# ninjasource/lc3-codec

Hardware: AMD Instinct MI355X
Metric: LC3 frames/sec (encode+decode) @48kHz/10ms (higher is better)
Workload: dtype f32

## Files before the change

### lc3-codec_amd/csrc/lc3_dev_common.h

```cpp
#pragma once
#include <stddef.h>
#include <stdint.h>

#include "lc3_dev_experiments.h"

#define LC3_TABLE_QUAL static __device__ const
#include "../../tables/lc3_tables.h"

#ifndef LC3_STAMP
#define LC3_STAMP(L, lane, id)
#endif

#ifndef LC3_CFG_PARAM
#define LC3_CFG_TEMPLATE
#define LC3_CFG_TEMPLATE_AND(...) template <__VA_ARGS__>
#define LC3_CFG_PARAM const lc3_cfg &c
#define LC3_CFG_BIND
#define LC3_CFG_PASS c
#endif

#ifndef LC3_LDS_PARAM
#define LC3_LDS_DECL(T, arr)
#define LC3_LDS_PARAM(T) T &L,
#define LC3_LDS_PASS L,
// ... 14 lines not shown
            (void)sub;
#define LC3_SERIAL_END \
        }              \
        LC3_SYNC();    \
    }
#endif
#ifndef LC3_SERIAL_WIDE_BEGIN
#define LC3_SERIAL_WIDE_BEGIN(T, L, lane, phase, K) LC3_SERIAL_BEGIN(T, L, lane, phase, K)
#endif

#define LC3_LOCAL_BEGIN(lane, K)    \
    {                               \
        LC3_SYNC();                 \
        if ((lane) < (K)) {         \
            const int sub = (lane); \
            (void)sub;
#define LC3_LOCAL_END \
        }             \
        LC3_SYNC();   \
    }

#ifndef LC3_KEEP_SCALAR
#define LC3_KEEP_SCALAR(x) ((void)0)
#endif
#ifndef LC3_UNIFORM_I32
#define LC3_UNIFORM_I32(x) (x)
#endif
#ifndef LC3_KEEP_PER_FRAME
#define LC3_KEEP_PER_FRAME(x) ((void)0)
#endif
#ifndef LC3_UNIFORM_PTR
#define LC3_UNIFORM_PTR(T, p) ((T)(p))
#endif
#ifndef LC3_LDS_BASE
#define LC3_LDS_BASE(p) (p)
#endif
#ifndef LC3_LDS_BASE_ALIGNED
#define LC3_LDS_BASE_ALIGNED(p, bytes) (p)
#endif
#ifndef LC3_HBM_CONST
#define LC3_HBM_CONST(T) const T *
#define LC3_HBM(T) T *
#endif

#define LC3_WAVE 64
#ifndef LC3_LOCKSTEP
// ... 885 lines not shown
```

### lc3-codec_amd/csrc/lc3_dev_enc.h

```cpp
#pragma once
#include "lc3_dev_common.h"
#include "lc3_dev_enc_pack.h"
#include "lc3_dev_enc_vq.h"

struct lc3_enc_scalars {
    float att_energy_last, att_max_energy_last;
    int att_pos_last, att_ds_tm1, att_ds_tm2;
    int t_prev;
    float mem_pitch;
    int mem_ltpf_active;
    float mem_nc, mem_mem_nc, h50_m1, h50_m2;
    int reset_offset_old;
    float nbits_offset_old;
    int nbits_est_old;
    int nbits_spec_old;
    int ring12_head, ring6_head, pad_[2];
};
struct lc3_enc_state {
    float x12[384];
    float x6[180];
    int16_t hist[304];
    lc3_enc_scalars sc;
};
static_assert(sizeof(lc3_enc_scalars) == 80 && sizeof(lc3_enc_state) % 16 == 0 && offsetof(lc3_enc_state, sc) % 16 == 0,
// ... 1 lines not shown

struct __attribute__((aligned(16))) lc3_enc_lds {
    lc3_enc_scalars st;
    float spec[LC3_MAX_NF];
    lc3_cpx fa[LC3_MAX_NF / 2];
    lc3_cpx fb[LC3_MAX_NF / 2];
    int16_t t[2 * LC3_MAX_NF];
    float sm[32];
    int ism[64];
    int spec_flags;
    int pad_;
    unsigned long long prof_last;
#ifdef LC3_PROFILE
    unsigned long long prof_acc[32];
#endif
};
#define LC3_ENC_DBG_EB 1472
#define LC3_ENC_DBG_ATTACK 1536
#define LC3_ENC_DBG_FLOATS 1600
#define LC3_EB(L) ((float *)(L).fa + 512)
#define LC3_SCF(L) ((float *)(L).fa + 144)
#define LC3_XQ(L) ((L).t)
#define LC3_RESW(L) ((uint32_t *)((uint8_t *)(L).t + 1024))

LC3_LDS_DECL(lc3_enc_lds, lc3_enc_wg)
static_assert(offsetof(lc3_enc_lds, fa) % 16 == 0 && offsetof(lc3_enc_lds, spec) % 16 == 0 && offsetof(lc3_enc_lds, t) % 16 == 0,
              "128-bit LDS reads need aligned buffers");
#ifndef LC3_PROFILE
static_assert(sizeof(lc3_enc_lds) <= 8192, "encoder working set: 8 KB per stream (the kernels run 16 waves per CU, register-bound)");
#endif

struct lc3_tns_res { int nbits_tns, lpc_weighting, num_tns_filters; int rc_order[2]; };
struct lc3_ltpf_res { int pitch_index, pitch_present, ltpf_active, nbits_ltpf; };
struct lc3_quant_res { int gg_ind, nbits_spec, nbits_lsb, nbits_trunc, lsb_mode, rate_flag, lastnz_trunc; float gg; };

#ifndef LC3_HBM_FENCE
#define LC3_HBM_FENCE() LC3_SYNC()
#endif

__device__ __forceinline__ void lc3_enc_state_init(lc3_enc_lds &L, int lane, lc3_enc_state *g, int valid) {
    int *w = (int *)&L.st;
    if (lane < (int)(sizeof(lc3_enc_scalars) / 4)) w[lane] = 0;
    if (valid) {
        int *gw = (int *)g;
        for (int i = lane; i < (int)(offsetof(lc3_enc_state, sc) / 4); i += LC3_WAVE) gw[i] = 0;
    }
// ... 333 lines not shown
        if (attack) {
            sSCF[0] = (sDS[0] + sDS[1] + sDS[2]) / 3.0f;
            sSCF[1] = (sDS[0] + sDS[1] + sDS[2] + sDS[3]) / 4.0f;
            for (int n = 2; n < 14; n++) {
                float wt = 0.0f;
                for (int k = n - 2; k < n + 3; k++) wt += sDS[k];
                sSCF[n] = wt / 5.0f;
            }
            sSCF[14] = (sDS[12] + sDS[13] + sDS[14] + sDS[15]) / 4.0f;
            sSCF[15] = (sDS[13] + sDS[14] + sDS[15]) / 3.0f;
            total = 0.0f;
            for (int n = 0; n < 16; n++) total += sSCF[n];
            avg = total / 16.0f;
            const float att = c.n_ms_10 ? 0.5f : 0.3f;
            for (int n = 0; n < 16; n++) sSCF[n] = att * (sSCF[n] - avg);
        } else {
            for (int n = 0; n < 16; n++) sSCF[n] = sDS[n];
        }
    }
    LC3_SYNC();
    LC3_STAMP(L, lane, 27);
}

#define LC3_TNS_CHUNK 4
struct lc3_tns_slot {
    float q[54];
    float es[6];
    int p_bw, near_nyquist, on[2];
    float rc[16];
};
static_assert(sizeof(lc3_tns_slot) * LC3_TNS_CHUNK <= sizeof(((lc3_enc_lds *)0)->fb), "the slots live in fb, which the back half does not use otherwise");
#define LC3_TNS_SLOT(L, u) (((lc3_tns_slot *)(L).fb)[(u)])

LC3_CFG_TEMPLATE __device__ __noinline__ void lc3_enc_tns_acf(LC3_CFG_PARAM, LC3_LDS_PARAM(lc3_enc_lds) int lane, int p_bw, int near_nyquist,
                                              int slot) {
    LC3_CFG_BIND;
    LC3_LDS_BIND(lc3_enc_lds, lc3_enc_wg);
    const lc3_tns_params &tp = c.n_ms_10 ? LC3C_TNS10[p_bw] : LC3C_TNS75[p_bw];
    lc3_tns_slot &T = LC3_TNS_SLOT(L, slot);
    float *sAC = T.q, *sES = T.es;
    float *x = L.spec;
    const int ne = c.ne;
    LC3_ENC_REPEAT(16) {
    if ((lane & 31) < 27) {
        const int j = (lane & 31) / 9, k = (lane & 31) - 9 * j;
        const int blk = lane < 32 ? (j == 2 ? 3 : j) : (j == 0 ? 2 : j + 3);
        const int f = blk >= 3, s = blk - 3 * f;
        float ac = 0.0f;
        if (f < tp.num) {
            const int start = tp.sub_start[f][s], stop = tp.sub_stop[f][s], k_from = start + k;
            if (k_from < ne && k_from < stop) {
                const float *pa = x + start, *pb = x + k_from;
                const int n = stop - k_from;
                for (int i = 0; i < n; i += 8) {
                    float xa[8], xb[8];
#pragma unroll
                    for (int u = 0; u < 8; u++) {
                        xa[u] = pa[i + u];
                        xb[u] = pb[i + u];
                    }
                    if (i + 8 <= n) {
#pragma unroll
                        for (int u = 0; u < 8; u++) ac += xa[u] * xb[u];
                    } else {
#pragma unroll
                        for (int u = 0; u < 8; u++) {
                            const float p = xa[u] * xb[u];
                            ac = i + u < n ? ac + p : ac;
                        }
                    }
                }
            }
        }
        sAC[f * 27 + k * 3 + s] = ac;
        if (k == 0) sES[f * 3 + s] = ac;
    }
    if (lane == 0) {
        T.p_bw = p_bw;
        T.near_nyquist = near_nyquist;
    }
    LC3_SYNC();
    if (lane < 54) {
        const int f = lane / 27, r = lane - 27 * f, s3 = r - 3 * (r / 3);
        sAC[lane] = sAC[lane] / sES[f * 3 + s3];
    }
    LC3_SYNC();
    }
    LC3_STAMP(L, lane, 28);
}

LC3_CFG_TEMPLATE __device__ __noinline__ void lc3_enc_tns_lev(LC3_CFG_PARAM, LC3_LDS_PARAM(lc3_enc_lds) int lane, int nbits, int n) {
    LC3_CFG_BIND;
    LC3_LDS_BIND(lc3_enc_lds, lc3_enc_wg);
    const int lpc_weighting = c.n_ms_10 ? (nbits < 480) : (nbits < 360);
    LC3_ENC_REPEAT(32)
    if (lane < 2 * n) {
        const int f = lane & 1;
        lc3_tns_slot &T = LC3_TNS_SLOT(L, lane >> 1);
        const float *sAC = T.q, *sES = T.es;
        float *rc_q = T.rc;
        const int num_g = (c.n_ms_10 ? LC3C_TNS10[T.p_bw] : LC3C_TNS75[T.p_bw]).num;
        int on = 0;
        if (f < num_g) {
        float r[9];
        const float e_prod = (1.0f * sES[f * 3] * sES[f * 3 + 1]) * sES[f * 3 + 2];
#pragma unroll
        for (int k = 0; k < 9; k++) {
            const float r0 = k == 0 ? 3.0f : 0.0f;
            const float rk = ((0.0f + sAC[f * 27 + k * 3]) + sAC[f * 27 + k * 3 + 1]) + sAC[f * 27 + k * 3 + 2];
            r[k] = (e_prod == 0.0f ? r0 : rk) * LC3C_TNS_LAGW[k];
        }
// ... 760 lines not shown
            LC3_GUARD_ASSERT((acc <= fits && nbits_spec >= 0) == ((int)lc3_ceilf((float)acc / 2048.0f) <= nbits_spec));
            cand_k = ok ? k0 + j : cand_k;
            cand_est = ok ? acc : cand_est;
        }
        const int best_k = lc3_wave_max_i32(cand_k, lane);
        const uint32_t best_est = best_k >= 0 ? (uint32_t)lc3_wave_read_i32((int)cand_est, best_k >> 2, lane) : 0u;
        bc.lastnz = lastnz;
        bc.lastnz_trunc = best_k < 0 ? 2 : 2 * best_k + 2;
        bc.nbits_est = (int)lc3_ceilf((float)est_total / 2048.0f) + (int)lsb_total;
        bc.nbits_trunc = (int)lc3_ceilf((float)best_est / 2048.0f);
        bc.nbits_lsb = (int)lsb_total;
    }
    (void)ntup_all;
    bc.rate_flag = rate_flag;
    bc.mode_flag = mode_flag;
    LC3_SYNC();
    for (int n = bc.lastnz_trunc + lane; n < bc.lastnz; n += LC3_WAVE) LC3_XQ(L)[n] = 0;
    LC3_SYNC();
    bc.lsb_mode = bc.mode_flag && bc.nbits_est > nbits_spec;
    bc.gg = gg;
    return bc;
}

LC3_CFG_TEMPLATE __device__ __noinline__ lc3_quant_res lc3_enc_quant(LC3_CFG_PARAM, LC3_LDS_PARAM(lc3_enc_lds) int lane, int nbits, int nbits_bw,
                                                      int nbits_tns, int nbits_ltpf) {
    LC3_CFG_BIND;
    LC3_LDS_BIND(lc3_enc_lds, lc3_enc_wg);
    const int ne = c.ne, ne4 = ne / 4;
    lc3_quant_res res;
    int nbits_ari = 0;
    while ((1 << nbits_ari) < ne / 2) nbits_ari++;
    nbits_ari += nbits <= 1280 ? 3 : (nbits <= 2560 ? 4 : 5);
    const int nbits_spec = nbits - (nbits_bw + nbits_tns + nbits_ltpf + 38 + 8 + 3 + nbits_ari);
    float nbits_offset;
    if (L.st.reset_offset_old) nbits_offset = 0.0f;
    else {
        float prev = L.st.nbits_offset_old + (float)L.st.nbits_spec_old - (float)L.st.nbits_est_old;
        nbits_offset = 0.8f * L.st.nbits_offset_old + 0.2f * lc3_minf(40.0f, lc3_maxf(-40.0f, prev));
    }
    const int nbits_spec_adj = lc3_f2u16((float)nbits_spec + nbits_offset + 0.5f);
    int gg_off;
    {
        int q = (int)(int16_t)nbits / (10 * (c.fs_ind + 1));
        gg_off = -(q < 115 ? q : 115) - 105 - 5 * (c.fs_ind + 1);
    }
    float e14[2], e28[2], amax = 0.0f;
    const lc3_divisor by20 = lc3_divisor_make(20.0f);
    LC3_ENC_REPEAT(1)
#pragma unroll
    for (int q = 0; q < 2; q++) {
        const int n = lane + LC3_WAVE * q;
        const lc3_f4 x = *(const lc3_f4 *)(L.spec + 4 * (n < ne4 ? n : 0));
// ... 85 lines not shown
        if (L.spec_flags & LC3_SPEC_NBITS_SPEC_OLD) L.st.nbits_spec_old = nbits_spec;
        L.st.reset_offset_old = reset_offset;
    }
    {
        const int t1 = LC3C_GGA_T1[c.fs_ind], t2 = LC3C_GGA_T2[c.fs_ind], t3 = LC3C_GGA_T3[c.fs_ind], est = bc.nbits_est, origin = gg_ind;
        float delta;
        if (est < t1) delta = ((float)est + 48.0f) / 16.0f;
        else if (est < t2) {
            float tmp1 = (float)t1 / 16.0f + 3.0f, tmp2 = (float)t2 / 48.0f;
            delta = ((float)est - (float)t1) * (tmp2 - tmp1) / ((float)t2 - (float)t1) + tmp1;
        } else if (est < t3) delta = (float)est / 48.0f;
        else delta = (float)t3 / 48.0f;
        delta = lc3_floorf(delta + 0.5f);
        const float delta2 = delta + 2.0f;
        if ((gg_ind < 255 && est > nbits_spec) || (gg_ind > 0 && (float)est < ((float)nbits_spec - delta2))) {
            if ((float)est < ((float)nbits_spec - delta2)) gg_ind -= 1;
            else if (gg_ind == 254 || (float)est < ((float)nbits_spec + delta)) gg_ind += 1;
            else gg_ind += 2;
            if (gg_ind < gg_min) gg_ind = gg_min;
        }
        if (origin != gg_ind)
            LC3_ENC_REPEAT(8) bc = lc3_quantize_spectrum(LC3_CFG_PASS, LC3_LDS_PASS lane, nbits, gg_off, gg_ind, nbits_spec);
    }
    res.gg_ind = gg_ind;
    res.nbits_spec = nbits_spec;
    res.nbits_lsb = bc.nbits_lsb;
    res.lsb_mode = bc.lsb_mode;
    res.nbits_trunc = bc.nbits_trunc;
    res.rate_flag = bc.rate_flag;
    res.lastnz_trunc = bc.lastnz_trunc;
    res.gg = bc.gg;
    return res;
}

LC3_CFG_TEMPLATE __device__ __noinline__ int lc3_enc_residual_noise(LC3_CFG_PARAM, LC3_LDS_PARAM(lc3_enc_lds) int lane,
                                                    const lc3_quant_res q, int bw_ind) {
    LC3_CFG_BIND;
    LC3_LDS_BIND(lc3_enc_lds, lc3_enc_wg);
    const int ne = c.ne;
    float *compact = (float *)L.fa;
    const int bw_stop = c.n_ms_10 ? LC3C_BWSTOP10[bw_ind] : LC3C_BWSTOP75[bw_ind];
    const int nf_start = c.n_ms_10 ? 24 : 18, nf_width = c.n_ms_10 ? 3 : 2;
    const int nf_stop = ne < bw_stop ? ne : bw_stop;
    int mx = q.nbits_spec - q.nbits_trunc + 4;
    if (mx < 0) mx = 0;
    const int k0 = 8 * lane;
    int xv[8];
    float sv[8];
    {
        const lc3_i4 w = *(const lc3_i4 *)(LC3_XQ(L) + k0);
        const lc3_f4 sa = *(const lc3_f4 *)(L.spec + k0), sb = *(const lc3_f4 *)(L.spec + k0 + 4);
        int wi[4];
        __builtin_memcpy(wi, &w, 16);
#pragma unroll
        for (int i = 0; i < 4; i++) {
// ... 220 lines not shown
        float *d = dbg + 1440;
        d[0] = (float)bw_ind; d[1] = (float)attack; d[9] = (float)pf.pitch_index; d[10] = (float)pf.pitch_present;
        d[11] = (float)pf.ltpf_active; d[21] = (float)near_nyquist;
        float *a = dbg + LC3_ENC_DBG_ATTACK;
        a[0] = L.st.att_energy_last; a[1] = L.st.att_max_energy_last; a[2] = (float)L.st.att_pos_last;
        a[3] = (float)L.st.att_ds_tm1; a[4] = (float)L.st.att_ds_tm2;
    }
    if (plane && mid && lane == 0) {
        const int st = plane_stride;
        int32_t *mf = (int32_t *)mid + MP_FLAGS;
        mf[MPF_BW] = bw_ind;
        mf[MPF_NBITS_BW] = nbits_bw;
        mf[MPF_NEAR_NYQUIST] = near_nyquist;
        mf[MPF_NBITS_LTPF] = pf.nbits_ltpf;
        plane[EP_BW * st] = bw_ind;
        plane[EP_NBITS_BW * st] = nbits_bw;
        plane[EP_PITCH_PRESENT * st] = pf.pitch_present;
        plane[EP_LTPF_ACTIVE * st] = pf.ltpf_active;
        plane[EP_PITCH_INDEX * st] = pf.pitch_index;
    }
    LC3_SYNC();
}

struct lc3_mid_fetch {
    lc3_i4 u[2];
    uint32_t bands[2];
    float g;
    int32_t flag;
};
template <class CC>
__device__ __forceinline__ void lc3_mid_issue(const CC &c, int lane, const float *mid, lc3_mid_fetch &m) {
    LC3_HBM_CONST(lc3_i4) s4 = (LC3_HBM_CONST(lc3_i4))(mid + MP_SPEC);
    const int n4 = c.ne / 4;
#pragma unroll
    for (int j = 0; j < 2; j++) {
        const int i = lane + LC3_WAVE * j;
        if (i < n4) {
            m.u[j] = s4[i];
            m.bands[j] = ((LC3_HBM_CONST(uint32_t))c.line_band)[i];
        }
    }
    m.g = lane < c.nb ? ((LC3_HBM_CONST(float))mid)[MP_G + lane] : 0.0f;
    m.flag = lane < 4 ? ((LC3_HBM_CONST(int32_t))mid)[MP_FLAGS + lane] : 0;
}

struct lc3_back_res {
    lc3_tns_res tns;
    lc3_quant_res spec;
    int n_res, noise_factor;
};
LC3_CFG_TEMPLATE __device__ __forceinline__ void lc3_encode_back_pickup(LC3_CFG_PARAM, lc3_enc_lds &L, int lane, const lc3_mid_fetch &m) {
    LC3_CFG_BIND;
    LC3_STAMP(L, lane, 0);
    float *gs = (float *)L.fa;
    if (lane < 4) L.ism[lane] = m.flag;
    if (lane < c.nb) gs[lane] = m.g;
    LC3_SYNC();
    LC3_ENC_REPEAT(128) {
        const int n4 = c.ne / 4;
#pragma unroll
        for (int j = 0; j < 2; j++) {
            const int i = lane + LC3_WAVE * j;
            if (i < n4) {
                const lc3_f4 xin = __builtin_bit_cast(lc3_f4, m.u[j]);
                float x[4] = {xin.x, xin.y, xin.z, xin.w};
                float gk[4];
#pragma unroll
                for (int q = 0; q < 4; q++) {
                    const uint32_t b = (m.bands[j] >> (8 * q)) & 0xffu;
                    gk[q] = gs[b < 64u ? b : 0u];
                }
#pragma unroll
                for (int q = 0; q < 4; q++) {
                    const uint32_t b = (m.bands[j] >> (8 * q)) & 0xffu;
                    x[q] = b < 64u ? x[q] * gk[q] : x[q];
                }
                lc3_f4 o;
                o.x = x[0]; o.y = x[1]; o.z = x[2]; o.w = x[3];
                ((lc3_f4 *)L.spec)[i] = o;
            }
        }
    }
    LC3_SYNC();
}
LC3_CFG_TEMPLATE __device__ __forceinline__ lc3_back_res lc3_encode_back_analyse(LC3_CFG_PARAM, lc3_enc_lds &L, int lane, int nbytes, int slot,
                                                                float *dbg) {
    LC3_CFG_BIND;
    const int nbits = nbytes * 8;
    const int bw_ind = L.ism[MPF_BW], nbits_bw = L.ism[MPF_NBITS_BW];
    const int nbits_ltpf = L.ism[MPF_NBITS_LTPF];
    LC3_STAMP(L, lane, 18);
    LC3_STAMP(L, lane, 19);
    if (dbg) for (int i = lane; i < c.nf; i += LC3_WAVE) dbg[480 + i] = L.spec[i];
    lc3_tns_res tns = {};
    if (LC3_KO(LC3_ENC_KO, 256)) tns.nbits_tns = 2, tns.num_tns_filters = 2;
    else tns = lc3_enc_tns_apply(LC3_CFG_PASS, LC3_LDS_PASS lane, bw_ind, nbits, slot);
    LC3_STAMP(L, lane, 4);
    if (dbg) for (int i = lane; i < c.nf; i += LC3_WAVE) dbg[960 + i] = L.spec[i];
    lc3_quant_res spec = {};
    if (LC3_KO(LC3_ENC_KO, 512)) spec.lastnz_trunc = 2, spec.gg = 1.0f;
    else spec = lc3_enc_quant(LC3_CFG_PASS, LC3_LDS_PASS lane, nbits, nbits_bw, tns.nbits_tns, nbits_ltpf);
    LC3_STAMP(L, lane, 6);
    int rn = LC3_KO(LC3_ENC_KO, 1024) ? 0 : lc3_enc_residual_noise(LC3_CFG_PASS, LC3_LDS_PASS lane, spec, bw_ind);
    LC3_ENC_REPEAT_MORE(64) rn = lc3_enc_residual_noise(LC3_CFG_PASS, LC3_LDS_PASS lane, spec, bw_ind);
    LC3_STAMP(L, lane, 7);
    lc3_back_res out;
    out.tns = tns;
    out.spec = spec;
    out.n_res = rn & 0xffff;
    out.noise_factor = rn >> 16;
    return out;
}
LC3_CFG_TEMPLATE __device__ __forceinline__ void lc3_encode_back_store(LC3_CFG_PARAM, lc3_enc_lds &L, int lane, const lc3_back_res &r,
                                                      int32_t *plane, int plane_stride, int store, float *dbg) {
    LC3_CFG_BIND;
    const lc3_tns_res &tns = r.tns;
    const lc3_quant_res &spec = r.spec;
    const int n_res = r.n_res, noise_factor = r.noise_factor;
    if (dbg && lane == 0) {
        float *d = dbg + 1440;
        const int st = plane_stride;
        d[2] = (float)plane[EP_IND_LF * st]; d[3] = (float)plane[EP_IND_HF * st];
        d[4] = (float)plane[EP_SHAPE_J * st]; d[5] = (float)plane[EP_GIND * st];
        d[6] = (float)tns.rc_order[0]; d[7] = (float)tns.rc_order[1]; d[8] = (float)tns.nbits_tns;
        d[12] = (float)spec.gg_ind; d[13] = (float)spec.lastnz_trunc;
        d[14] = (float)spec.nbits_lsb; d[15] = (float)spec.lsb_mode; d[16] = (float)n_res; d[17] = (float)noise_factor;
        d[18] = spec.gg; d[19] = (float)spec.nbits_spec; d[20] = (float)spec.nbits_trunc;
        const uint32_t joint = (uint32_t)plane[EP_JOINT * st];
        d[22] = (float)plane[EP_LS_INDA * st]; d[23] = (float)(joint & 0xffffu); d[24] = (float)(joint >> 16);
    }
    if (store) {
        const int st = plane_stride;
        if (lane == 0) {
            plane[EP_LASTNZ_TRUNC * st] = spec.lastnz_trunc;
            plane[EP_LSB_MODE * st] = spec.lsb_mode;
            plane[EP_GG_IND * st] = spec.gg_ind;
            plane[EP_NUM_TNS * st] = tns.num_tns_filters;
            plane[EP_ORD0 * st] = tns.rc_order[0];
            plane[EP_ORD1 * st] = tns.rc_order[1];
            plane[EP_LPC_W * st] = tns.lpc_weighting;
            plane[EP_NOISE * st] = noise_factor;
            plane[EP_RATE_FLAG * st] = spec.rate_flag;
            plane[EP_N_RES * st] = n_res;
        }
        if (lane < 16) plane[(EP_RCI + lane) * st] = L.ism[16 + lane];
        if (lane < 13) plane[(EP_RES + lane) * st] = (int32_t)LC3_RESW(L)[lane];
        if (LC3_PLANE_STRIDE == 1) lc3_wave_copy_out16(plane + EP_XQ, LC3_XQ(L), (c.ne / 2 + 3) / 4, lane);
        else
            for (int k = lane; k < c.ne / 2; k += LC3_WAVE)
                plane[(EP_XQ + k) * st] = (int32_t)(((uint32_t)(uint16_t)LC3_XQ(L)[2 * k]) | ((uint32_t)(uint16_t)LC3_XQ(L)[2 * k + 1] << 16));
        if (L.spec_flags & LC3_LAUNCH_PREP_SYMBOLS) lc3_enc_symbols(LC3_CFG_PASS, LC3_LDS_PASS lane, spec, plane, st);
        else if (lane == 0) plane[EP_NSYM * st] = -1;
    }
    LC3_SYNC();
    LC3_STAMP(L, lane, 8);
}
LC3_CFG_TEMPLATE __device__ __forceinline__ void lc3_encode_back_stream(LC3_CFG_PARAM, lc3_enc_lds &L, int lane, const float *mid, int32_t *planes,
                                                       size_t fbase, int n_frames, int nbytes, int store, float *dbg) {
    LC3_CFG_BIND;
    lc3_mid_fetch cur, nxt;
    if (n_frames > 0) lc3_mid_issue(c, lane, mid + fbase * (size_t)MP_WORDS, cur);
    nxt = cur;
    for (int t0 = 0; t0 < n_frames; t0 += LC3_TNS_CHUNK) {
        const int nc = n_frames - t0 < LC3_TNS_CHUNK ? n_frames - t0 : LC3_TNS_CHUNK;
        if (nc > 1) {
            for (int u = 0; u < nc; u++) {
                const int tn = u + 1 < nc ? t0 + u + 1 : t0;
                lc3_mid_issue(c, lane, mid + (fbase + (size_t)tn) * (size_t)MP_WORDS, nxt);
                lc3_encode_back_pickup(LC3_CFG_PASS, L, lane, cur);
                lc3_enc_tns_acf(LC3_CFG_PASS, LC3_LDS_PASS lane, L.ism[MPF_BW], L.ism[MPF_NEAR_NYQUIST], u);
                cur = nxt;
            }
            lc3_enc_tns_lev(LC3_CFG_PASS, LC3_LDS_PASS lane, nbytes * 8, nc);
        }
        for (int u = 0; u < nc; u++) {
            const int t = t0 + u;
            if (t + 1 < n_frames) lc3_mid_issue(c, lane, mid + (fbase + (size_t)t + 1) * (size_t)MP_WORDS, nxt);
            lc3_encode_back_pickup(LC3_CFG_PASS, L, lane, cur);
            if (nc == 1) {
                lc3_enc_tns_acf(LC3_CFG_PASS, LC3_LDS_PASS lane, L.ism[MPF_BW], L.ism[MPF_NEAR_NYQUIST], 0);
                lc3_enc_tns_lev(LC3_CFG_PASS, LC3_LDS_PASS lane, nbytes * 8, 1);
            }
            const lc3_back_res r = lc3_encode_back_analyse(LC3_CFG_PASS, L, lane, nbytes, u, dbg);
            lc3_encode_back_store(LC3_CFG_PASS, L, lane, r, LC3_PLANE_COL(planes, fbase + (size_t)t, EP_WORDS), LC3_PLANE_STRIDE, store, dbg);
            cur = nxt;
        }
    }
}
```

### lc3-codec_amd/csrc/lc3_dev_enc_vbr.h

```cpp
#ifndef LC3_DEV_ENC_VBR_H_
#define LC3_DEV_ENC_VBR_H_

#define LC3_VBR_MIN_BYTES 20

__device__ __forceinline__ int lc3_vbr_enc_size(const uint16_t *nb, size_t idx, int slot, int *clamped) {
    const int v = (int)nb[idx];
    const int lo = LC3_VBR_MIN_BYTES;
    *clamped = v < lo || v > slot;
    return v < lo ? lo : (v > slot ? slot : v);
}
__device__ __forceinline__ int lc3_vbr_enc_size(const uint16_t *nb, size_t idx, int slot) {
    int unused;
    return lc3_vbr_enc_size(nb, idx, slot, &unused);
}

template <class CC>
__device__ __forceinline__ int lc3_vbr_gain_ltpf_on(const CC &c, int nbytes) {
    const int nbits = nbytes * 8;
    int t_nbits = nbits;
    if (!c.n_ms_10) {
        double v = (double)nbits * 10.0 / 7.5;
        t_nbits = (int)(v + 0.5);
    }
    return t_nbits < 560 + c.fs_ind * 80;
}

template <class CC>
__device__ __forceinline__ int lc3_vbr_front_phase(const CC &c, const uint16_t *nb, int slot, int wg_s0, int n_streams, int t, int n_frames,
                                                   int n_waves) {
    int phase = t % n_waves;
    if (t + 2 >= n_frames) return phase;
    int off = 0;
    for (int w = 0; w < n_waves; w++) {
        const int s_raw = wg_s0 + w, s = s_raw < n_streams ? s_raw : n_streams - 1;
        for (int u = t; u <= t + 2; u++) off |= lc3_vbr_gain_ltpf_on(c, lc3_vbr_enc_size(nb, (size_t)s * (size_t)n_frames + (size_t)u, slot));
    }
    return phase + (off ? 0 : 0x100);
}

template <class CC>
__device__ __forceinline__ int lc3_vbr_lpc_weighting(const CC &c, int nbytes) {
    const int nbits = nbytes * 8;
    return c.n_ms_10 ? (nbits < 480) : (nbits < 360);
}

LC3_CFG_TEMPLATE __device__ __forceinline__ void lc3_encode_back_stream_vbr(LC3_CFG_PARAM, lc3_enc_lds &L, int lane, const float *mid,
                                                                           int32_t *planes, size_t fbase, int n_frames, const uint16_t *nb_row,
                                                                           int slot, int store, float *dbg) {
    LC3_CFG_BIND;
    lc3_mid_fetch cur, nxt;
    if (n_frames > 0) lc3_mid_issue(c, lane, mid + fbase * (size_t)MP_WORDS, cur);
    nxt = cur;
    for (int t0 = 0; t0 < n_frames;) {
        const int nb0 = lc3_vbr_enc_size(nb_row, (size_t)t0, slot);
        const int w0 = lc3_vbr_lpc_weighting(c, nb0);
        int nc = 1;
        while (nc < LC3_TNS_CHUNK && t0 + nc < n_frames && lc3_vbr_lpc_weighting(c, lc3_vbr_enc_size(nb_row, (size_t)(t0 + nc), slot)) == w0) nc++;
        if (nc > 1) {
            for (int u = 0; u < nc; u++) {
                const int tn = u + 1 < nc ? t0 + u + 1 : t0;
                lc3_mid_issue(c, lane, mid + (fbase + (size_t)tn) * (size_t)MP_WORDS, nxt);
                lc3_encode_back_pickup(LC3_CFG_PASS, L, lane, cur);
                lc3_enc_tns_acf(LC3_CFG_PASS, LC3_LDS_PASS lane, L.ism[MPF_BW], L.ism[MPF_NEAR_NYQUIST], u);
                cur = nxt;
            }
            lc3_enc_tns_lev(LC3_CFG_PASS, LC3_LDS_PASS lane, nb0 * 8, nc);
        }
        for (int u = 0; u < nc; u++) {
            const int t = t0 + u;
            const int nbt = lc3_vbr_enc_size(nb_row, (size_t)t, slot);
            if (t + 1 < n_frames) lc3_mid_issue(c, lane, mid + (fbase + (size_t)t + 1) * (size_t)MP_WORDS, nxt);
            lc3_encode_back_pickup(LC3_CFG_PASS, L, lane, cur);
            if (nc == 1) {
                lc3_enc_tns_acf(LC3_CFG_PASS, LC3_LDS_PASS lane, L.ism[MPF_BW], L.ism[MPF_NEAR_NYQUIST], 0);
                lc3_enc_tns_lev(LC3_CFG_PASS, LC3_LDS_PASS lane, nbt * 8, 1);
            }
            const lc3_back_res r = lc3_encode_back_analyse(LC3_CFG_PASS, L, lane, nbt, u, dbg);
            lc3_encode_back_store(LC3_CFG_PASS, L, lane, r, LC3_PLANE_COL(planes, fbase + (size_t)t, EP_WORDS), LC3_PLANE_STRIDE, store, dbg);
            cur = nxt;
        }
        t0 += nc;
    }
}

#endif
```

### lc3-codec_amd/csrc/lc3_dev_experiments.h

```cpp
#pragma once

#ifndef LC3_ENC_KO
#define LC3_ENC_KO 0
#endif
#ifndef LC3_ENC_DUP
#define LC3_ENC_DUP 0
#endif
#define LC3_KO(set, bit) (((set) & (bit)) != 0)
#ifndef LC3_EXP_TWO
#define LC3_EXP_TWO() 2
#endif
#ifndef LC3_EXP_CLOBBER
#define LC3_EXP_CLOBBER() ((void)0)
#endif
#define LC3_EXP_REPS(set, bit) ((((set) & (bit)) != 0) ? LC3_EXP_TWO() : 1)
#if LC3_ENC_DUP
#define LC3_ENC_REPEAT(bit) for (int rep_ = LC3_EXP_REPS(LC3_ENC_DUP, bit); rep_ > 0; rep_--, LC3_EXP_CLOBBER())
#define LC3_ENC_REPEAT_MORE(bit) for (int rep_ = LC3_EXP_REPS(LC3_ENC_DUP, bit); rep_ > 1; rep_--, LC3_EXP_CLOBBER())
#else
#define LC3_ENC_REPEAT(bit)
#define LC3_ENC_REPEAT_MORE(bit) if (false)
#endif
```

### lc3-codec_amd/csrc/lc3gpu.hip

```cpp
#include <hip/hip_runtime.h>

#include <cmath>
#include <cstdio>
#include <cstdlib>
#include <cstring>
#include <algorithm>
#include <mutex>
#include <new>
#include <vector>

#include "../../include/lc3gpu.h"

#ifdef LC3_TU_KIND
#define LC3_MULTI_TU 1
#ifndef LC3_TU_INDEX
#define LC3_TU_INDEX 0
#endif
#else
#define LC3_MULTI_TU 0
#define LC3_TU_KIND 0
#define LC3_TU_INDEX 0
#endif
#if LC3_TU_KIND == 0
#define LC3_TU_STATIC
// ... 86 lines not shown
#define LC3_SERIAL_END \
        }              \
        LC3_SERIAL_PRIO_DOWN(); \
        __syncthreads(); \
    }
#define LC3_SERIAL_WIDE_BEGIN(T, L, lane, phase, K)                                                           \
    {                                                                                                         \
        T *lc3_wg_base_ = &(L) - LC3_WAVE_ID();                                                               \
        __syncthreads();                                                                                      \
        const int lc3_v_ = (lane) + 64 * ((LC3_WAVE_ID() + LC3_WG_WAVES - ((phase) % LC3_WG_WAVES)) % LC3_WG_WAVES); \
        if (lc3_v_ - (lane) < LC3_WG_WAVES * (K)) LC3_SERIAL_PRIO_UP();                                       \
        if (lc3_v_ < LC3_WG_WAVES * (K)) {                                                                    \
            T &L = lc3_wg_base_[lc3_v_ / (K)];                                                                \
            const int sub = lc3_v_ % (K);                                                                     \
            (void)sub;
#endif
#define LC3_HBM_CONST(T) const __attribute__((address_space(1))) T *
#define LC3_HBM(T) __attribute__((address_space(1))) T *
#define LC3_UNIFORM_I32(x) __builtin_amdgcn_readfirstlane((int)(x))
#define LC3_UNIFORM_PTR(T, p)                                                                                             \
    ((T)(((unsigned long long)(unsigned)__builtin_amdgcn_readfirstlane((int)((unsigned long long)(uintptr_t)(p) >> 32)) << 32) | \
         (unsigned long long)(unsigned)__builtin_amdgcn_readfirstlane((int)(unsigned)(uintptr_t)(p))))
#define LC3_KEEP_SCALAR(x) asm("" : "+v"(x))
static __device__ __forceinline__ const float *lc3_lds_base(const float *p) {
    unsigned a = (unsigned)(uintptr_t)(const __attribute__((address_space(3))) float *)p;
    asm("" : "+v"(a));
    return (const float *)(const __attribute__((address_space(3))) float *)(uintptr_t)a;
}
#define LC3_LDS_BASE(p) lc3_lds_base(p)
template <unsigned BYTES>
static __device__ __forceinline__ const float *lc3_lds_base_aligned(const float *p) {
    unsigned a = (unsigned)(uintptr_t)(const __attribute__((address_space(3))) float *)p;
    asm("" : "+v"(a));
    a &= ~(BYTES - 1u);
    return (const float *)(const __attribute__((address_space(3))) float *)(uintptr_t)a;
}
#define LC3_LDS_BASE_ALIGNED(p, bytes) lc3_lds_base_aligned<bytes>(p)
#define LC3_KEEP_PER_FRAME(x) asm volatile("" : "+v"(x))
static __device__ __forceinline__ int lc3_exp_two() {
    int n = 2;
    asm volatile("" : "+s"(n) : : "memory");
    return n;
}
#define LC3_EXP_TWO() lc3_exp_two()
static __device__ __forceinline__ void lc3_exp_clobber() { asm volatile("" : : : "memory"); }
#define LC3_EXP_CLOBBER() lc3_exp_clobber()
// ... 5215 lines not shown
```

Before: 59.83 million.

## Overlap next-frame prefetch and deferred output flush with encoder back-half compute

```diff
diff --git a/lc3-codec_amd/csrc/lc3_dev_common.h b/lc3-codec_amd/csrc/lc3_dev_common.h
--- a/lc3-codec_amd/csrc/lc3_dev_common.h
+++ b/lc3-codec_amd/csrc/lc3_dev_common.h
@@ -60,6 +60,9 @@
 
 #ifndef LC3_KEEP_SCALAR
 #define LC3_KEEP_SCALAR(x) ((void)0)
+#endif
+#ifndef LC3_LOADED
+#define LC3_LOADED(a, b) ((void)0)
 #endif
 #ifndef LC3_UNIFORM_I32
 #define LC3_UNIFORM_I32(x) (x)
diff --git a/lc3-codec_amd/csrc/lc3_dev_enc.h b/lc3-codec_amd/csrc/lc3_dev_enc.h
--- a/lc3-codec_amd/csrc/lc3_dev_enc.h
+++ b/lc3-codec_amd/csrc/lc3_dev_enc.h
@@ -47,6 +47,8 @@
 #define LC3_SCF(L) ((float *)(L).fa + 144)
 #define LC3_XQ(L) ((L).t)
 #define LC3_RESW(L) ((uint32_t *)((uint8_t *)(L).t + 1024))
+#define LC3_COLW(L) ((int32_t *)((uint8_t *)(L).t + 1088))
+static_assert(1088 + 4 * EP_XQ <= sizeof(((lc3_enc_lds *)0)->t), "quantised spectrum, residual bits and the column head share t");
 
 LC3_LDS_DECL(lc3_enc_lds, lc3_enc_wg)
 static_assert(offsetof(lc3_enc_lds, fa) % 16 == 0 && offsetof(lc3_enc_lds, spec) % 16 == 0 && offsetof(lc3_enc_lds, t) % 16 == 0,
@@ -426,6 +428,35 @@
     LC3_STAMP(L, lane, 27);
 }
 
+struct lc3_mid_fetch {
+    lc3_i4 u[2];
+    float g;
+    int32_t flag;
+};
+template <class CC>
+__device__ __forceinline__ void lc3_mid_issue(const CC &c, int lane, const float *mid, lc3_mid_fetch &m) {
+    LC3_HBM_CONST(lc3_i4) s4 = (LC3_HBM_CONST(lc3_i4))(mid + MP_SPEC);
+    const int n4 = c.ne / 4;
+#pragma unroll
+    for (int j = 0; j < 2; j++) {
+        const int i = lane + LC3_WAVE * j;
+        if (i < n4) m.u[j] = s4[i];
+    }
+    m.g = lane < c.nb ? ((LC3_HBM_CONST(float))mid)[MP_G + lane] : 0.0f;
+    m.flag = lane < 4 ? ((LC3_HBM_CONST(int32_t))mid)[MP_FLAGS + lane] : 0;
+}
+struct lc3_mid_bands { uint32_t w[2]; };
+template <class CC>
+__device__ __forceinline__ lc3_mid_bands lc3_mid_bands_load(const CC &c, int lane) {
+    lc3_mid_bands b;
+#pragma unroll
+    for (int j = 0; j < 2; j++) {
+        const int i = lane + LC3_WAVE * j;
+        b.w[j] = i < c.ne / 4 ? ((LC3_HBM_CONST(uint32_t))c.line_band)[i] : 0u;
+    }
+    return b;
+}
+
 #define LC3_TNS_CHUNK 4
 struct lc3_tns_slot {
     float q[54];
@@ -436,8 +467,8 @@
 static_assert(sizeof(lc3_tns_slot) * LC3_TNS_CHUNK <= sizeof(((lc3_enc_lds *)0)->fb), "the slots live in fb, which the back half does not use otherwise");
 #define LC3_TNS_SLOT(L, u) (((lc3_tns_slot *)(L).fb)[(u)])
 
-LC3_CFG_TEMPLATE __device__ __noinline__ void lc3_enc_tns_acf(LC3_CFG_PARAM, LC3_LDS_PARAM(lc3_enc_lds) int lane, int p_bw, int near_nyquist,
-                                              int slot) {
+LC3_CFG_TEMPLATE __device__ __noinline__ lc3_mid_fetch lc3_enc_tns_acf(LC3_CFG_PARAM, LC3_LDS_PARAM(lc3_enc_lds) int lane, int p_bw, int near_nyquist,
+                                                       int slot, const float *mid_next) {
     LC3_CFG_BIND;
     LC3_LDS_BIND(lc3_enc_lds, lc3_enc_wg);
     const lc3_tns_params &tp = c.n_ms_10 ? LC3C_TNS10[p_bw] : LC3C_TNS75[p_bw];
@@ -445,14 +476,21 @@
     float *sAC = T.q, *sES = T.es;
     float *x = L.spec;
     const int ne = c.ne;
+    const int summing = (lane & 31) < 27;
+    const int j = summing ? (lane & 31) / 9 : 0, k = (lane & 31) - 9 * j;
+    const int blk = lane < 32 ? (j == 2 ? 3 : j) : (j == 0 ? 2 : j + 3);
+    const int f = blk >= 3, s = blk - 3 * f;
+    const int has_filter = f < tp.num;
+    int start = 0, stop = 0;
+    if (summing && has_filter) start = tp.sub_start[f][s], stop = tp.sub_stop[f][s];
+    LC3_LOADED(start, stop);
+    lc3_mid_fetch next;
+    lc3_mid_issue(c, lane, mid_next, next);
     LC3_ENC_REPEAT(16) {
-    if ((lane & 31) < 27) {
-        const int j = (lane & 31) / 9, k = (lane & 31) - 9 * j;
-        const int blk = lane < 32 ? (j == 2 ? 3 : j) : (j == 0 ? 2 : j + 3);
-        const int f = blk >= 3, s = blk - 3 * f;
+    if (summing) {
         float ac = 0.0f;
-        if (f < tp.num) {
-            const int start = tp.sub_start[f][s], stop = tp.sub_stop[f][s], k_from = start + k;
+        if (has_filter) {
+            const int k_from = start + k;
             if (k_from < ne && k_from < stop) {
                 const float *pa = x + start, *pb = x + k_from;
                 const int n = stop - k_from;
@@ -491,6 +529,7 @@
     LC3_SYNC();
     }
     LC3_STAMP(L, lane, 28);
+    return next;
 }
 
 LC3_CFG_TEMPLATE __device__ __noinline__ void lc3_enc_tns_lev(LC3_CFG_PARAM, LC3_LDS_PARAM(lc3_enc_lds) int lane, int nbits, int n) {
@@ -1297,12 +1336,54 @@
     return bc;
 }
 
-LC3_CFG_TEMPLATE __device__ __noinline__ lc3_quant_res lc3_enc_quant(LC3_CFG_PARAM, LC3_LDS_PARAM(lc3_enc_lds) int lane, int nbits, int nbits_bw,
-                                                      int nbits_tns, int nbits_ltpf) {
+#define LC3_COL_BACK_WORDS                                                                                                                   \
+    ((1ull << EP_LASTNZ_TRUNC) | (1ull << EP_LSB_MODE) | (1ull << EP_GG_IND) | (1ull << EP_NUM_TNS) | (1ull << EP_ORD0) | (1ull << EP_ORD1) | \
+     (1ull << EP_LPC_W) | (1ull << EP_NOISE) | (1ull << EP_RATE_FLAG) | (1ull << EP_N_RES) | (0xffffull << EP_RCI) | (0x1fffull << EP_RES))
+static_assert(EP_XQ <= 64, "one lane per word of the column head");
+LC3_CFG_TEMPLATE __device__ __forceinline__ void lc3_encode_back_flush(LC3_CFG_PARAM, lc3_enc_lds &L, int lane, int32_t *plane) {
+    LC3_CFG_BIND;
+    const int st = LC3_PLANE_STRIDE;
+    LC3_HBM(int32_t) col = (LC3_HBM(int32_t))plane;
+    const unsigned long long words = LC3_COL_BACK_WORDS | ((L.spec_flags & LC3_LAUNCH_PREP_SYMBOLS) ? 0ull : 1ull << EP_NSYM);
+    if ((words >> lane) & 1ull) col[lane * st] = LC3_COLW(L)[lane];
+    if (LC3_PLANE_STRIDE == 1) {
+        LC3_HBM(lc3_i4) d = (LC3_HBM(lc3_i4))(col + EP_XQ);
+        const lc3_i4 *s = (const lc3_i4 *)LC3_XQ(L);
+        for (int i = lane; i < (c.ne / 2 + 3) / 4; i += LC3_WAVE) d[i] = s[i];
+    } else {
+        for (int k = lane; k < c.ne / 2; k += LC3_WAVE)
+            col[(EP_XQ + k) * st] = (int32_t)(((uint32_t)(uint16_t)LC3_XQ(L)[2 * k]) | ((uint32_t)(uint16_t)LC3_XQ(L)[2 * k + 1] << 16));
+    }
+}
+
+struct lc3_quant_out {
+    lc3_mid_fetch next;
+    int gg_ind_lastnz;
+    int lsb_rate;
+    int nbits_spec, nbits_lsb, nbits_trunc;
+    float gg;
+};
+__device__ __forceinline__ lc3_quant_res lc3_quant_out_res(const lc3_quant_out &o) {
+    lc3_quant_res r;
+    r.gg_ind = o.gg_ind_lastnz >> 16;
+    r.lastnz_trunc = o.gg_ind_lastnz & 0xffff;
+    r.lsb_mode = o.lsb_rate & 1;
+    r.rate_flag = o.lsb_rate & 512;
+    r.nbits_spec = o.nbits_spec;
+    r.nbits_lsb = o.nbits_lsb;
+    r.nbits_trunc = o.nbits_trunc;
+    r.gg = o.gg;
+    return r;
+}
+
+LC3_CFG_TEMPLATE __device__ __noinline__ lc3_quant_out lc3_enc_quant(LC3_CFG_PARAM, LC3_LDS_PARAM(lc3_enc_lds) int lane, int nbits, int nbits_bw,
+                                                      int nbits_tns, int nbits_ltpf, const float *mid_next, int32_t *flush) {
     LC3_CFG_BIND;
     LC3_LDS_BIND(lc3_enc_lds, lc3_enc_wg);
     const int ne = c.ne, ne4 = ne / 4;
-    lc3_quant_res res;
+    lc3_quant_out out;
+    lc3_mid_issue(c, lane, mid_next, out.next);
+    if (flush) lc3_encode_back_flush(LC3_CFG_PASS, L, lane, flush);
     int nbits_ari = 0;
     while ((1 << nbits_ari) < ne / 2) nbits_ari++;
     nbits_ari += nbits <= 1280 ? 3 : (nbits <= 2560 ? 4 : 5);
@@ -1434,15 +1515,13 @@
         if (origin != gg_ind)
             LC3_ENC_REPEAT(8) bc = lc3_quantize_spectrum(LC3_CFG_PASS, LC3_LDS_PASS lane, nbits, gg_off, gg_ind, nbits_spec);
     }
-    res.gg_ind = gg_ind;
-    res.nbits_spec = nbits_spec;
-    res.nbits_lsb = bc.nbits_lsb;
-    res.lsb_mode = bc.lsb_mode;
-    res.nbits_trunc = bc.nbits_trunc;
-    res.rate_flag = bc.rate_flag;
-    res.lastnz_trunc = bc.lastnz_trunc;
-    res.gg = bc.gg;
-    return res;
+    out.gg_ind_lastnz = (bc.lastnz_trunc & 0xffff) | (int)((uint32_t)gg_ind << 16);
+    out.lsb_rate = bc.lsb_mode | bc.rate_flag;
+    out.nbits_spec = nbits_spec;
+    out.nbits_lsb = bc.nbits_lsb;
+    out.nbits_trunc = bc.nbits_trunc;
+    out.gg = bc.gg;
+    return out;
 }
 
 LC3_CFG_TEMPLATE __device__ __noinline__ int lc3_enc_residual_noise(LC3_CFG_PARAM, LC3_LDS_PARAM(lc3_enc_lds) int lane,
@@ -1709,34 +1788,13 @@
     LC3_SYNC();
 }
 
-struct lc3_mid_fetch {
-    lc3_i4 u[2];
-    uint32_t bands[2];
-    float g;
-    int32_t flag;
-};
-template <class CC>
-__device__ __forceinline__ void lc3_mid_issue(const CC &c, int lane, const float *mid, lc3_mid_fetch &m) {
-    LC3_HBM_CONST(lc3_i4) s4 = (LC3_HBM_CONST(lc3_i4))(mid + MP_SPEC);
-    const int n4 = c.ne / 4;
-#pragma unroll
-    for (int j = 0; j < 2; j++) {
-        const int i = lane + LC3_WAVE * j;
-        if (i < n4) {
-            m.u[j] = s4[i];
-            m.bands[j] = ((LC3_HBM_CONST(uint32_t))c.line_band)[i];
-        }
-    }
-    m.g = lane < c.nb ? ((LC3_HBM_CONST(float))mid)[MP_G + lane] : 0.0f;
-    m.flag = lane < 4 ? ((LC3_HBM_CONST(int32_t))mid)[MP_FLAGS + lane] : 0;
-}
-
 struct lc3_back_res {
     lc3_tns_res tns;
     lc3_quant_res spec;
     int n_res, noise_factor;
 };
-LC3_CFG_TEMPLATE __device__ __forceinline__ void lc3_encode_back_pickup(LC3_CFG_PARAM, lc3_enc_lds &L, int lane, const lc3_mid_fetch &m) {
+LC3_CFG_TEMPLATE __device__ __forceinline__ void lc3_encode_back_pickup(LC3_CFG_PARAM, lc3_enc_lds &L, int lane, const lc3_mid_fetch &m,
+                                                                       const lc3_mid_bands &bands) {
     LC3_CFG_BIND;
     LC3_STAMP(L, lane, 0);
     float *gs = (float *)L.fa;
@@ -1754,12 +1812,12 @@
                 float gk[4];
 #pragma unroll
                 for (int q = 0; q < 4; q++) {
-                    const uint32_t b = (m.bands[j] >> (8 * q)) & 0xffu;
+                    const uint32_t b = (bands.w[j] >> (8 * q)) & 0xffu;
                     gk[q] = gs[b < 64u ? b : 0u];
                 }
 #pragma unroll
                 for (int q = 0; q < 4; q++) {
-                    const uint32_t b = (m.bands[j] >> (8 * q)) & 0xffu;
+                    const uint32_t b = (bands.w[j] >> (8 * q)) & 0xffu;
                     x[q] = b < 64u ? x[q] * gk[q] : x[q];
                 }
                 lc3_f4 o;
@@ -1771,7 +1829,7 @@
     LC3_SYNC();
 }
 LC3_CFG_TEMPLATE __device__ __forceinline__ lc3_back_res lc3_encode_back_analyse(LC3_CFG_PARAM, lc3_enc_lds &L, int lane, int nbytes, int slot,
-                                                                float *dbg) {
+                                                                const float *mid_next, int32_t *flush, lc3_mid_fetch &next, float *dbg) {
     LC3_CFG_BIND;
     const int nbits = nbytes * 8;
     const int bw_ind = L.ism[MPF_BW], nbits_bw = L.ism[MPF_NBITS_BW];
@@ -1785,8 +1843,15 @@
     LC3_STAMP(L, lane, 4);
     if (dbg) for (int i = lane; i < c.nf; i += LC3_WAVE) dbg[960 + i] = L.spec[i];
     lc3_quant_res spec = {};
-    if (LC3_KO(LC3_ENC_KO, 512)) spec.lastnz_trunc = 2, spec.gg = 1.0f;
-    else spec = lc3_enc_quant(LC3_CFG_PASS, LC3_LDS_PASS lane, nbits, nbits_bw, tns.nbits_tns, nbits_ltpf);
+    if (LC3_KO(LC3_ENC_KO, 512)) {
+        spec.lastnz_trunc = 2, spec.gg = 1.0f;
+        lc3_mid_issue(c, lane, mid_next, next);
+        if (flush) lc3_encode_back_flush(LC3_CFG_PASS, L, lane, flush);
+    } else {
+        const lc3_quant_out q = lc3_enc_quant(LC3_CFG_PASS, LC3_LDS_PASS lane, nbits, nbits_bw, tns.nbits_tns, nbits_ltpf, mid_next, flush);
+        spec = lc3_quant_out_res(q);
+        next = q.next;
+    }
     LC3_STAMP(L, lane, 6);
     int rn = LC3_KO(LC3_ENC_KO, 1024) ? 0 : lc3_enc_residual_noise(LC3_CFG_PASS, LC3_LDS_PASS lane, spec, bw_ind);
     LC3_ENC_REPEAT_MORE(64) rn = lc3_enc_residual_noise(LC3_CFG_PASS, LC3_LDS_PASS lane, spec, bw_ind);
@@ -1798,7 +1863,7 @@
     out.noise_factor = rn >> 16;
     return out;
 }
-LC3_CFG_TEMPLATE __device__ __forceinline__ void lc3_encode_back_store(LC3_CFG_PARAM, lc3_enc_lds &L, int lane, const lc3_back_res &r,
+LC3_CFG_TEMPLATE __device__ __forceinline__ void lc3_encode_back_stage(LC3_CFG_PARAM, lc3_enc_lds &L, int lane, const lc3_back_res &r,
                                                       int32_t *plane, int plane_stride, int store, float *dbg) {
     LC3_CFG_BIND;
     const lc3_tns_res &tns = r.tns;
@@ -1817,60 +1882,77 @@
         d[22] = (float)plane[EP_LS_INDA * st]; d[23] = (float)(joint & 0xffffu); d[24] = (float)(joint >> 16);
     }
     if (store) {
-        const int st = plane_stride;
+        int32_t *w = LC3_COLW(L);
         if (lane == 0) {
-            plane[EP_LASTNZ_TRUNC * st] = spec.lastnz_trunc;
-            plane[EP_LSB_MODE * st] = spec.lsb_mode;
-            plane[EP_GG_IND * st] = spec.gg_ind;
-            plane[EP_NUM_TNS * st] = tns.num_tns_filters;
-            plane[EP_ORD0 * st] = tns.rc_order[0];
-            plane[EP_ORD1 * st] = tns.rc_order[1];
-            plane[EP_LPC_W * st] = tns.lpc_weighting;
-            plane[EP_NOISE * st] = noise_factor;
-            plane[EP_RATE_FLAG * st] = spec.rate_flag;
-            plane[EP_N_RES * st] = n_res;
-        }
-        if (lane < 16) plane[(EP_RCI + lane) * st] = L.ism[16 + lane];
-        if (lane < 13) plane[(EP_RES + lane) * st] = (int32_t)LC3_RESW(L)[lane];
-        if (LC3_PLANE_STRIDE == 1) lc3_wave_copy_out16(plane + EP_XQ, LC3_XQ(L), (c.ne / 2 + 3) / 4, lane);
-        else
-            for (int k = lane; k < c.ne / 2; k += LC3_WAVE)
-                plane[(EP_XQ + k) * st] = (int32_t)(((uint32_t)(uint16_t)LC3_XQ(L)[2 * k]) | ((uint32_t)(uint16_t)LC3_XQ(L)[2 * k + 1] << 16));
-        if (L.spec_flags & LC3_LAUNCH_PREP_SYMBOLS) lc3_enc_symbols(LC3_CFG_PASS, LC3_LDS_PASS lane, spec, plane, st);
-        else if (lane == 0) plane[EP_NSYM * st] = -1;
+            w[EP_LASTNZ_TRUNC] = spec.lastnz_trunc;
+            w[EP_LSB_MODE] = spec.lsb_mode;
+            w[EP_GG_IND] = spec.gg_ind;
+            w[EP_NUM_TNS] = tns.num_tns_filters;
+            w[EP_ORD0] = tns.rc_order[0];
+            w[EP_ORD1] = tns.rc_order[1];
+            w[EP_LPC_W] = tns.lpc_weighting;
+            w[EP_NOISE] = noise_factor;
+            w[EP_RATE_FLAG] = spec.rate_flag;
+            w[EP_N_RES] = n_res;
+            w[EP_NSYM] = -1;
+        }
+        if (lane < 16) w[EP_RCI + lane] = L.ism[16 + lane];
+        if (lane < 13) w[EP_RES + lane] = (int32_t)LC3_RESW(L)[lane];
+        if (L.spec_flags & LC3_LAUNCH_PREP_SYMBOLS) lc3_enc_symbols(LC3_CFG_PASS, LC3_LDS_PASS lane, spec, plane, plane_stride);
     }
     LC3_SYNC();
     LC3_STAMP(L, lane, 8);
 }
-LC3_CFG_TEMPLATE __device__ __forceinline__ void lc3_encode_back_stream(LC3_CFG_PARAM, lc3_enc_lds &L, int lane, const float *mid, int32_t *planes,
-                                                       size_t fbase, int n_frames, int nbytes, int store, float *dbg) {
+struct lc3_back_uniform {
+    int nb;
+    __device__ __forceinline__ int nbytes(int) const { return nb; }
+    template <class CC>
+    __device__ __forceinline__ int chunk(const CC &, int t0, int n_frames) const {
+        return n_frames - t0 < LC3_TNS_CHUNK ? n_frames - t0 : LC3_TNS_CHUNK;
+    }
+};
+LC3_CFG_TEMPLATE_AND(class SIZES)
+__device__ __forceinline__ void lc3_encode_back_frames(LC3_CFG_PARAM, lc3_enc_lds &L, int lane, const float *mid, int32_t *planes, size_t fbase,
+                                                       int n_frames, const SIZES sizes, int store, float *dbg) {
     LC3_CFG_BIND;
-    lc3_mid_fetch cur, nxt;
+    const lc3_mid_bands bands = lc3_mid_bands_load(c, lane);
+    lc3_mid_fetch cur;
     if (n_frames > 0) lc3_mid_issue(c, lane, mid + fbase * (size_t)MP_WORDS, cur);
-    nxt = cur;
-    for (int t0 = 0; t0 < n_frames; t0 += LC3_TNS_CHUNK) {
-        const int nc = n_frames - t0 < LC3_TNS_CHUNK ? n_frames - t0 : LC3_TNS_CHUNK;
+    int32_t *staged = nullptr;
+    for (int t0 = 0; t0 < n_frames;) {
+        const int nc = sizes.chunk(c, t0, n_frames);
         if (nc > 1) {
             for (int u = 0; u < nc; u++) {
                 const int tn = u + 1 < nc ? t0 + u + 1 : t0;
-                lc3_mid_issue(c, lane, mid + (fbase + (size_t)tn) * (size_t)MP_WORDS, nxt);
-                lc3_encode_back_pickup(LC3_CFG_PASS, L, lane, cur);
-                lc3_enc_tns_acf(LC3_CFG_PASS, LC3_LDS_PASS lane, L.ism[MPF_BW], L.ism[MPF_NEAR_NYQUIST], u);
-                cur = nxt;
-            }
-            lc3_enc_tns_lev(LC3_CFG_PASS, LC3_LDS_PASS lane, nbytes * 8, nc);
+                lc3_encode_back_pickup(LC3_CFG_PASS, L, lane, cur, bands);
+                cur = lc3_enc_tns_acf(LC3_CFG_PASS, LC3_LDS_PASS lane, L.ism[MPF_BW], L.ism[MPF_NEAR_NYQUIST], u,
+                                      mid + (fbase + (size_t)tn) * (size_t)MP_WORDS);
+            }
+            lc3_enc_tns_lev(LC3_CFG_PASS, LC3_LDS_PASS lane, sizes.nbytes(t0) * 8, nc);
         }
         for (int u = 0; u < nc; u++) {
-            const int t = t0 + u;
-            if (t + 1 < n_frames) lc3_mid_issue(c, lane, mid + (fbase + (size_t)t + 1) * (size_t)MP_WORDS, nxt);
-            lc3_encode_back_pickup(LC3_CFG_PASS, L, lane, cur);
+            const int t = t0 + u, nbytes = sizes.nbytes(t);
+            const float *mid_next = mid + (fbase + (size_t)(t + 1 < n_frames ? t + 1 : t)) * (size_t)MP_WORDS;
+            lc3_encode_back_pickup(LC3_CFG_PASS, L, lane, cur, bands);
             if (nc == 1) {
-                lc3_enc_tns_acf(LC3_CFG_PASS, LC3_LDS_PASS lane, L.ism[MPF_BW], L.ism[MPF_NEAR_NYQUIST], 0);
+                lc3_enc_tns_acf(LC3_CFG_PASS, LC3_LDS_PASS lane, L.ism[MPF_BW], L.ism[MPF_NEAR_NYQUIST], 0, mid + (fbase + (size_t)t) * (size_t)MP_WORDS);
                 lc3_enc_tns_lev(LC3_CFG_PASS, LC3_LDS_PASS lane, nbytes * 8, 1);
             }
-            const lc3_back_res r = lc3_encode_back_analyse(LC3_CFG_PASS, L, lane, nbytes, u, dbg);
-            lc3_encode_back_store(LC3_CFG_PASS, L, lane, r, LC3_PLANE_COL(planes, fbase + (size_t)t, EP_WORDS), LC3_PLANE_STRIDE, store, dbg);
-            cur = nxt;
-        }
-    }
-}
+            const lc3_back_res r = lc3_encode_back_analyse(LC3_CFG_PASS, L, lane, nbytes, u, mid_next, staged, cur, dbg);
+            int32_t *plane = LC3_PLANE_COL(planes, fbase + (size_t)t, EP_WORDS);
+            lc3_encode_back_stage(LC3_CFG_PASS, L, lane, r, plane, LC3_PLANE_STRIDE, store, dbg);
+            staged = store ? plane : nullptr;
+            if (LC3_BACK_STORE_AT_END && staged) {
+                lc3_encode_back_flush(LC3_CFG_PASS, L, lane, staged);
+                staged = nullptr;
+            }
+        }
+        t0 += nc;
+    }
+    if (staged) lc3_encode_back_flush(LC3_CFG_PASS, L, lane, staged);
+}
+LC3_CFG_TEMPLATE __device__ __forceinline__ void lc3_encode_back_stream(LC3_CFG_PARAM, lc3_enc_lds &L, int lane, const float *mid, int32_t *planes,
+                                                       size_t fbase, int n_frames, int nbytes, int store, float *dbg) {
+    const lc3_back_uniform sizes = {nbytes};
+    lc3_encode_back_frames(LC3_CFG_PASS, L, lane, mid, planes, fbase, n_frames, sizes, store, dbg);
+}
diff --git a/lc3-codec_amd/csrc/lc3_dev_enc_vbr.h b/lc3-codec_amd/csrc/lc3_dev_enc_vbr.h
--- a/lc3-codec_amd/csrc/lc3_dev_enc_vbr.h
+++ b/lc3-codec_amd/csrc/lc3_dev_enc_vbr.h
@@ -44,43 +44,23 @@
     return c.n_ms_10 ? (nbits < 480) : (nbits < 360);
 }
 
+struct lc3_back_sized {
+    const uint16_t *nb_row;
+    int slot;
+    __device__ __forceinline__ int nbytes(int t) const { return lc3_vbr_enc_size(nb_row, (size_t)t, slot); }
+    template <class CC>
+    __device__ __forceinline__ int chunk(const CC &c, int t0, int n_frames) const {
+        const int w0 = lc3_vbr_lpc_weighting(c, nbytes(t0));
+        int nc = 1;
+        while (nc < LC3_TNS_CHUNK && t0 + nc < n_frames && lc3_vbr_lpc_weighting(c, nbytes(t0 + nc)) == w0) nc++;
+        return nc;
+    }
+};
 LC3_CFG_TEMPLATE __device__ __forceinline__ void lc3_encode_back_stream_vbr(LC3_CFG_PARAM, lc3_enc_lds &L, int lane, const float *mid,
                                                                            int32_t *planes, size_t fbase, int n_frames, const uint16_t *nb_row,
                                                                            int slot, int store, float *dbg) {
-    LC3_CFG_BIND;
-    lc3_mid_fetch cur, nxt;
-    if (n_frames > 0) lc3_mid_issue(c, lane, mid + fbase * (size_t)MP_WORDS, cur);
-    nxt = cur;
-    for (int t0 = 0; t0 < n_frames;) {
-        const int nb0 = lc3_vbr_enc_size(nb_row, (size_t)t0, slot);
-        const int w0 = lc3_vbr_lpc_weighting(c, nb0);
-        int nc = 1;
-        while (nc < LC3_TNS_CHUNK && t0 + nc < n_frames && lc3_vbr_lpc_weighting(c, lc3_vbr_enc_size(nb_row, (size_t)(t0 + nc), slot)) == w0) nc++;
-        if (nc > 1) {
-            for (int u = 0; u < nc; u++) {
-                const int tn = u + 1 < nc ? t0 + u + 1 : t0;
-                lc3_mid_issue(c, lane, mid + (fbase + (size_t)tn) * (size_t)MP_WORDS, nxt);
-                lc3_encode_back_pickup(LC3_CFG_PASS, L, lane, cur);
-                lc3_enc_tns_acf(LC3_CFG_PASS, LC3_LDS_PASS lane, L.ism[MPF_BW], L.ism[MPF_NEAR_NYQUIST], u);
-                cur = nxt;
-            }
-            lc3_enc_tns_lev(LC3_CFG_PASS, LC3_LDS_PASS lane, nb0 * 8, nc);
-        }
-        for (int u = 0; u < nc; u++) {
-            const int t = t0 + u;
-            const int nbt = lc3_vbr_enc_size(nb_row, (size_t)t, slot);
-            if (t + 1 < n_frames) lc3_mid_issue(c, lane, mid + (fbase + (size_t)t + 1) * (size_t)MP_WORDS, nxt);
-            lc3_encode_back_pickup(LC3_CFG_PASS, L, lane, cur);
-            if (nc == 1) {
-                lc3_enc_tns_acf(LC3_CFG_PASS, LC3_LDS_PASS lane, L.ism[MPF_BW], L.ism[MPF_NEAR_NYQUIST], 0);
-                lc3_enc_tns_lev(LC3_CFG_PASS, LC3_LDS_PASS lane, nbt * 8, 1);
-            }
-            const lc3_back_res r = lc3_encode_back_analyse(LC3_CFG_PASS, L, lane, nbt, u, dbg);
-            lc3_encode_back_store(LC3_CFG_PASS, L, lane, r, LC3_PLANE_COL(planes, fbase + (size_t)t, EP_WORDS), LC3_PLANE_STRIDE, store, dbg);
-            cur = nxt;
-        }
-        t0 += nc;
-    }
+    const lc3_back_sized sizes = {nb_row, slot};
+    lc3_encode_back_frames(LC3_CFG_PASS, L, lane, mid, planes, fbase, n_frames, sizes, store, dbg);
 }
 
 #endif
diff --git a/lc3-codec_amd/csrc/lc3_dev_experiments.h b/lc3-codec_amd/csrc/lc3_dev_experiments.h
--- a/lc3-codec_amd/csrc/lc3_dev_experiments.h
+++ b/lc3-codec_amd/csrc/lc3_dev_experiments.h
@@ -5,6 +5,9 @@
 #endif
 #ifndef LC3_ENC_DUP
 #define LC3_ENC_DUP 0
+#endif
+#ifndef LC3_BACK_STORE_AT_END
+#define LC3_BACK_STORE_AT_END 0
 #endif
 #define LC3_KO(set, bit) (((set) & (bit)) != 0)
 #ifndef LC3_EXP_TWO
diff --git a/lc3-codec_amd/csrc/lc3gpu.hip b/lc3-codec_amd/csrc/lc3gpu.hip
--- a/lc3-codec_amd/csrc/lc3gpu.hip
+++ b/lc3-codec_amd/csrc/lc3gpu.hip
@@ -132,6 +132,7 @@
     ((T)(((unsigned long long)(unsigned)__builtin_amdgcn_readfirstlane((int)((unsigned long long)(uintptr_t)(p) >> 32)) << 32) | \
          (unsigned long long)(unsigned)__builtin_amdgcn_readfirstlane((int)(unsigned)(uintptr_t)(p))))
 #define LC3_KEEP_SCALAR(x) asm("" : "+v"(x))
+#define LC3_LOADED(a, b) asm volatile("" : "+v"(a), "+v"(b) : : "memory")
 static __device__ __forceinline__ const float *lc3_lds_base(const float *p) {
     unsigned a = (unsigned)(uintptr_t)(const __attribute__((address_space(3))) float *)p;
     asm("" : "+v"(a));
```

After: 59.46 million. No clear change (-0.6%).
